# stefantaubert/waveglow

Hardware: AMD Instinct MI355X
Metric: audio samples/sec/GPU (22.05 kHz) WaveGlow-256 infer; real-time factor (higher is better)
Workload: dtype f16 MFMA operands, f32 accumulate/flow state, fp16 I/O; 1 GPU; configs[1]: 256ch WaveGlow.infer, batch=16/GPU mels 80x864, fp16 I/O, sigma=0.6; parallelism=utterance-sharded x1, no collective

## Files before the change

### waveglow_amd/csrc/kernels.hip

```cpp
#include "wg_common.h"

#include <cstdlib>
#include <type_traits>

namespace wg {

typedef _Float16 half8 __attribute__((ext_vector_type(8)));
typedef _Float16 half4 __attribute__((ext_vector_type(4)));
typedef float f32x16 __attribute__((ext_vector_type(16)));
typedef float f32x4 __attribute__((ext_vector_type(4)));

#define WG_GPTR(p) ((const __attribute__((address_space(1))) void*)(p))
#define WG_LPTR(p) ((__attribute__((address_space(3))) void*)(p))

__device__ __forceinline__ float load_io(const void* p, size_t i, int f16) {
  return f16 ? (float)((const _Float16*)p)[i] : ((const float*)p)[i];
}

__device__ __forceinline__ float gate_act(float u, float v) {
  const float e1 = __builtin_amdgcn_exp2f(__builtin_amdgcn_fmed3f(u, -60.0f, 60.0f));
  const float t = 1.0f + __builtin_amdgcn_exp2f(v);
  return (e1 - 1.0f) * __builtin_amdgcn_rcpf(fmaf(e1, t, t));
}

__device__ __forceinline__ void gate_act3(float u, float v, float& th, float& sg, float& ac) {
  const float e1 = __builtin_amdgcn_exp2f(__builtin_amdgcn_fmed3f(u, -60.0f, 60.0f));
  const float t = 1.0f + __builtin_amdgcn_exp2f(__builtin_amdgcn_fmed3f(v, -60.0f, 60.0f));
  const float r = __builtin_amdgcn_rcpf(fmaf(e1, t, t));
  ac = fmaf(e1, r, -r);
  sg = fmaf(e1, r, r);
  th = ac * t;
}

__device__ __forceinline__ void glds16(const void* sbase, unsigned voff, unsigned lds_addr) {
  unsigned keep;
  asm volatile("s_mov_b32 %0, m0\n\ts_mov_b32 m0, %3\n\ts_nop 2\n\tglobal_load_lds_dwordx4 %1, %2\n\ts_mov_b32 m0, %0"
               : "=&s"(keep) : "v"(voff), "s"(sbase), "s"(lds_addr) : "memory");
}
template <int OFF>
__device__ __forceinline__ void gload16(half8& dst, const void* sbase, unsigned voff) {
  asm volatile("s_nop 4\n\tglobal_load_dwordx4 %0, %1, %2 offset:%3" : "=v"(dst) : "v"(voff), "s"(sbase), "i"(OFF) : "memory");
}

#ifdef WG_STAMPS
#define WG_STAMP(i)                                                                              \
  do {                                                                                           \
    __builtin_amdgcn_sched_barrier(0);                                                           \
    unsigned long long _t;                                                                       \
    asm volatile("s_memtime %0\n\ts_waitcnt lgkmcnt(0)" : "=s"(_t)::"memory");                   \
    if (a.stamps && HAS_RES && tid == 0) a.stamps[(size_t)tile * 8 + (i)] = _t;                        \
    __builtin_amdgcn_sched_barrier(0);                                                           \
  } while (0)
#else
#define WG_STAMP(i) do {} while (0)
#endif

constexpr int kTilesPerWG = 2;


__device__ __forceinline__ void mfma16_acc(f32x4& c, const half8& a, const half8& b) {
  c = __builtin_amdgcn_mfma_f32_16x16x32_f16(a, b, c, 0, 0, 0);
}

template <int C> struct WnCfg {
  static constexpr int NW = (C >= 256) ? 8 : C / 32;
  static constexpr int BN = (C >= 512) ? 64 : 128;
};

template <int N> __device__ __forceinline__ void wait_vm() {
  asm volatile("s_waitcnt vmcnt(%0)" :: "i"(N) : "memory");
  __builtin_amdgcn_sched_barrier(0);
}

template <int C, int NW, int BN, bool HAS_RES, int TPW, int CX, int MODE = 0, int NTAPS = 3, bool HAS_COND = true, bool DEEP = false, bool M16 = false>
__global__ void __launch_bounds__(NW * 64) wn_layer_kernel(const WnLayerArgs a) {
  constexpr bool TR = MODE == 1;
  constexpr bool PLAIN = MODE >= 2;
  constexpr int MB = C / (32 * NW);
  constexpr int MT = PLAIN ? MB : 2 * MB;
  constexpr int NTHREADS = NW * 64;
  constexpr int NT = BN / 32;
  constexpr int CC = CX;
  constexpr int NKX = NTAPS * CC;
  constexpr int BT_BYTES = BN * 128;
  constexpr int ACT_ROW = 2 * C + 16;
  constexpr int K2 = C / 16;
  constexpr int NG = BN * 8 / NTHREADS;
  constexpr int NAH = MT * 2;
  constexpr bool DEFER = (MB == 1);
  static_assert(BN * 8 % NTHREADS == 0 && MB >= 1 && MB <= 2 && NKX >= 1 && (NTAPS == 1 || NTAPS == 3), "tile geometry");
  constexpr bool Q2L = !M16 && DEFER && !DEEP && (NG + NT - 1) / NT == 1 && NT >= NG + MT;
  static_assert(!M16 || (MODE == 0 && MB == 1 && DEFER && !DEEP && NT >= 2), "16x16x32 variant");
  constexpr bool A0G = MODE == 0 && CX == 1 && NTAPS == 1;
  static_assert(!DEEP || (MODE == 0 && DEFER && HAS_COND && MT <= NT && NG <= NT && ((NKX >= 4 && NKX % 2 == 0) || NKX == 1)), "deep prefetch variant");
  static_assert(MODE == 0 || (TPW == 1 && CX == ((MODE == 2 || MODE == 4) ? 2 : 1) * (C / 64)) || (MODE == 3 && CX == 1), "training variants");

  extern __shared__ __attribute__((aligned(16))) char smem[];
  char* const sB = smem;
  char* const sActs = MODE == 4 ? smem : smem + 2 * BT_BYTES;

  const int tid = threadIdx.x;
  const int wave = __builtin_amdgcn_readfirstlane(tid >> 6);
  int lane = tid & 63, ln = lane & 31, lh = lane >> 5;

  unsigned pvoff[NG];
  int pchunk[NG];
  int swB;
  int l15 = lane & 15, l4 = lane >> 4;
  unsigned a_voff;
  auto set_lane_ids = [&]() {
    int t = tid;
    asm volatile("" : "+v"(t));
    lane = t & 63;
    ln = lane & 31;
    lh = lane >> 5;
    swB = M16 ? (lane >> 1) & 7 : (ln >> 1) & 7;
    l15 = lane & 15;
    l4 = lane >> 4;
    a_voff = lane * 16;
#pragma unroll
    for (int i = 0; i < NG; ++i) {
      const int idx = i * NTHREADS + t;
      const int row = idx >> 3, pc = idx & 7;
      pchunk[i] = pc ^ ((row >> 1) & 7);
      pvoff[i] = row * 128 + (pchunk[i] << 4);
    }
  };
  set_lane_ids();
  const unsigned sB_addr = (unsigned)(size_t)WG_LPTR(sB);
  const int R = a.g.R, Rp = a.g.Rp, Fp = a.g.Fp, M = a.M;
  const int nK = NKX + (HAS_COND ? a.n_cond_steps : 0);
  const int mel_rows_per_utt = a.g.T + 6;

  auto xstep_src = [&](int p, int jt, int ks) -> const char* {
    const int tap = ks / CC, cc = ks - tap * CC;
    const int pp = p + (tap - NTAPS / 2) * a.dil;
    const int row = kRowPad + (pp & 31) * Rp + a.row0 + jt * BN + (pp >> 5);
    return (const char*)(a.x_tap + ((size_t)cc * R + row) * 64);
  };
  auto sp_src = [&](int p, int jt, int s_) -> const char* {
    const int row = kRowPad + p * Rp + a.row0 + jt * BN;
    return (const char*)(a.sp + ((size_t)s_ * R + row) * 64);
  };
  int mrow[NG];
  auto cond_voff = [&](int s, int i) -> unsigned {
    const int k0 = s * 64 + pchunk[i] * 8;
    const int j = (k0 >= M) + (k0 >= 2 * M) + (k0 >= 3 * M);
    return (unsigned)(((mrow[i] - j) * M + (k0 - j * M)) * 2);
  };
  auto stage_B_piece = [&](int p, int jt, int ks, int bufsel, int i) {
    const unsigned lds = __builtin_amdgcn_readfirstlane(sB_addr + bufsel * BT_BYTES + (i * NTHREADS + wave * 64) * 16);
    if constexpr (A0G) {
      if (ks < NKX) {
        const int row = (i * NTHREADS + tid) >> 3, lc = pchunk[i];
        const int pp = p + ((lc < 3 ? lc : 1) - 1) * a.dil;
        const unsigned prow = (unsigned)(kRowPad + (pp & 31) * Rp + a.row0 + jt * BN + (pp >> 5) + row);
        glds16(a.x_tap, prow * 128u + (lc < 3 ? 0u : (unsigned)lc * 16u), lds);
        return;
      }
    }
    if (ks < NKX) glds16(xstep_src(p, jt, ks), pvoff[i], lds);
    else if constexpr (MODE != 0) glds16(sp_src(p, jt, ks - NKX), pvoff[i], lds);
    else glds16(a.melT, cond_voff(ks - NKX, i), lds);
  };
  auto read_B = [&](const char* buf, int nt, int k16) -> half8 {
    const int n = nt * 32 + ln;
    const int c = (k16 * 2 + lh) ^ swB;
    return *(const half8*)(buf + n * 128 + c * 16);
  };
  auto read_B16 = [&](const char* buf, int g, int nt) -> half8 {
    const int n = (NT * (g & 1) + nt) * 16 + l15;
    const int c = (4 * (g >> 1) + l4) ^ swB;
    return *(const half8*)(buf + n * 128 + c * 16);
  };
  const char* wA1c_p = nullptr;
  auto load_Aq = [&](int ks, int g, int mt, half8& dst) {
    const char* base = ks < NKX ? (const char*)a.wA1 : wA1c_p;
    const int kl = ks < NKX ? ks : ks - NKX;
    const char* p = base + ((size_t)(2 * kl + (g >> 1)) * NW + wave) * (NAH * 1024) + (mt * 2 + (g & 1)) * 1024;
    gload16<0>(dst, p, a_voff);
  };
  auto load_A16 = [&](int ks, int s_, int m, half8& dst) {
    const char* base = ks < NKX ? (const char*)a.wA1 : wA1c_p;
    const int kl = ks < NKX ? ks : ks - NKX;
    gload16<0>(dst, base + ((size_t)(2 * kl + s_) * NW + wave) * (NAH * 1024) + m * 1024, a_voff);
  };
  int tile_b0 = 0;
  const bool fp_ge_bn = Fp >= BN;
  auto column_of = [&](int rr, int p, int& b, int& t) -> bool {
    int rem = rr - tile_b0 * Fp;
    b = tile_b0;
    if (fp_ge_bn) {
      if (rem >= Fp) { rem -= Fp; ++b; }
    } else {
      const int qd = rem / Fp;
      b += qd;
      rem -= qd * Fp;
    }
    const int fq = rem - a.g.Gf;
    t = fq * 32 + p;
    if (!(b < a.g.B && fq >= 0 && fq < a.g.F && t < a.g.L)) return false;
    return a.g.frames == nullptr || t < 32 * a.g.frames[b];
  };

  int tile, tile_end;
  const int tile_step = gridDim.x >> 3;
  int run_start, run_quarter = 0;
  {
    const int bid = blockIdx.x, ntl = a.n_tiles;
    const int xcd = bid & 7, idx = bid >> 3;
    const int qq = ntl >> 3, r = ntl & 7;
    const int start = xcd < r ? xcd * (qq + 1) : r * (qq + 1) + (xcd - r) * qq;
    tile_end = start + (xcd < r ? qq + 1 : qq);
    tile = start + idx;
    run_start = start;
    if (((tile_end - start) & 3) == 0) run_quarter = (tile_end - start) >> 2;
  }
  auto tile_of = [&](int t) { return run_quarter ? run_start + ((t - run_start) & 3) * run_quarter + ((t - run_start) >> 2) : t; };

  half8 q[4][MT];
  int par = 0;
  if (tile < tile_end) {
    const int t0 = tile_of(tile), p0 = t0 / a.tiles_per_phase;
#pragma unroll
    for (int i = 0; i < NG; ++i) stage_B_piece(p0, t0 - p0 * a.tiles_per_phase, 0, 0, i);
  }
  float* const sBias = (float*)(sActs + BN * ACT_ROW);
  if constexpr (!PLAIN) {
    for (int i = tid; i < 2 * C; i += NTHREADS) sBias[i] = a.bias1[i];
    if constexpr (HAS_RES)
      for (int i = tid; i < C; i += NTHREADS) sBias[2 * C + i] = a.bias2[i];
    uint4* const sW = (uint4*)(sBias + 3 * C);
    for (int i = tid; i < (C / 32) * 64; i += NTHREADS) sW[i] = ((const uint4*)a.wEs)[i];
  }
  __syncthreads();

#pragma unroll
  for (int it = 0; it < TPW; ++it, tile += tile_step) {
    if (tile >= tile_end) break;
    if (it > 0) set_lane_ids();
    const int tile_m = tile_of(tile);
    const int p = tile_m / a.tiles_per_phase;
    const int jt = tile_m - p * a.tiles_per_phase;
    const int rr0 = a.row0 + jt * BN;
    tile_b0 = rr0 / Fp;
    const int r0 = kRowPad + p * Rp + rr0;
    const int next_tile = tile + tile_step;
    wA1c_p = (const char*)a.wA1c + (MODE != 0 ? (size_t)0 : (size_t)p * (2 * a.n_cond_steps) * NW * (NAH * 1024));
    half8 Q[DEEP ? 2 : 1][4][MT];
    if constexpr (DEEP) {
#pragma unroll
      for (int g = 0; g < 4; ++g)
#pragma unroll
        for (int mt = 0; mt < MT; ++mt) load_Aq(0, g, mt, Q[0][g][mt]);
#pragma unroll
      for (int g = 0; g < 2; ++g)
#pragma unroll
        for (int mt = 0; mt < MT; ++mt) load_Aq(1, g, mt, Q[DEEP ? 1 : 0][g][mt]);
    } else {
#pragma unroll
      for (int g = 0; g < (Q2L || M16 ? 2 : 3); ++g)
#pragma unroll
        for (int mt = 0; mt < MT; ++mt) {
          if constexpr (M16) load_A16(0, 0, 2 * g + mt, q[g][mt]);
          else load_Aq(0, g, mt, q[g][mt]);
        }
    }
    if constexpr (MODE == 0) {
#pragma unroll
      for (int i = 0; i < NG; ++i) {
        int b, t;
        const int rr = rr0 + ((i * NTHREADS + tid) >> 3);
        const bool ok = column_of(rr, p, b, t);
        mrow[i] = ok ? 3 + b * mel_rows_per_utt + 3 + (t >> 5) : 3;
      }
    }
    unsigned vmask = 0;
#pragma unroll
    for (int nt = 0; nt < NT; ++nt) {
      int cb, ct;
      vmask |= column_of(rr0 + nt * 32 + ln, p, cb, ct) ? (1u << nt) : 0u;
    }
    WG_STAMP(0);
    f32x16 acc[MT][NT];
    f32x4 acc4[M16 ? MT : 1][M16 ? NT : 1][4];
    auto acc_at = [&](int mt, int nt, int e) -> float {
      if constexpr (M16) return acc4[mt][nt][e >> 2][e & 3];
      else return acc[mt][nt][e];
    };
#pragma unroll
    for (int mt = 0; mt < MT; ++mt) {
      f32x16 v;
      if constexpr (PLAIN) {
#pragma unroll
        for (int j = 0; j < 16; ++j) v[j] = 0.0f;
      } else {
        const int row0 = (mt < MB ? 0 : C) + (wave * MB + (mt < MB ? mt : mt - MB)) * 32;
        const float4* bp = (const float4*)(sBias + row0 + 4 * (M16 ? l4 : lh));
#pragma unroll
        for (int g = 0; g < 4; ++g) {
          const float4 q4 = bp[M16 ? 4 * (g >> 1) : 2 * g];
          v[4 * g] = q4.x; v[4 * g + 1] = q4.y; v[4 * g + 2] = q4.z; v[4 * g + 3] = q4.w;
        }
      }
#pragma unroll
      for (int nt = 0; nt < NT; ++nt) {
        if constexpr (M16) {
#pragma unroll
          for (int e = 0; e < 4; ++e) acc4[mt][nt][e] = f32x4{v[4 * e], v[4 * e + 1], v[4 * e + 2], v[4 * e + 3]};
        } else {
          acc[mt][nt] = v;
        }
      }
    }

    constexpr bool PIPE = !PLAIN && HAS_RES && MB == 1;
    constexpr bool RES_A0 = A0G && wn_res_a0(C);
    half8 a2r[PIPE ? K2 : 1];
    wait_vm<DEEP ? 3 * MT : 0>();
    __builtin_amdgcn_s_barrier();
    __builtin_amdgcn_sched_barrier(0);
    WG_STAMP(1);
    constexpr int LPS = (MT + NT - 1) / NT;
    constexpr int GPS = (NG + NT - 1) / NT;
    half8 bf[2][NT];
    constexpr bool PRIO = NW == 8 && ((BN == 128 && ((MODE == 0 && CX == C / 64) || MODE == 1)) || (C == 512 && MODE == 0 && CX == C / 64));
    auto prio_set = [&](int hi_grp) {
      if (hi_grp == 1)
        asm volatile("s_cmp_lt_u32 %0, 4\n\ts_cbranch_scc1 .Lpa%=\n\ts_setprio 1\n\ts_branch .Lpb%=\n.Lpa%=:\n\ts_setprio 0\n.Lpb%=:" :: "s"(wave) : "memory", "scc");
      else
        asm volatile("s_cmp_lt_u32 %0, 4\n\ts_cbranch_scc1 .Lpa%=\n\ts_setprio 0\n\ts_branch .Lpb%=\n.Lpa%=:\n\ts_setprio 1\n.Lpb%=:" :: "s"(wave) : "memory", "scc");
    };
    auto mfma_col = [&](int g, int nt) {
      if constexpr (M16) {
        const int t16 = NT * (g & 1) + nt;
#pragma unroll
        for (int m = 0; m < 4; ++m) {
          mfma16_acc(acc4[m >> 1][t16 >> 1][2 * (m & 1) + (t16 & 1)], q[2 * (g >> 1) + (m >> 1)][m & 1], bf[g & 1][nt]);
        }
      } else {
#pragma unroll
        for (int mt = 0; mt < MT; ++mt) {
          acc[mt][nt] = __builtin_amdgcn_mfma_f32_32x32x16_f16(q[g][mt], bf[g & 1][nt], acc[mt][nt], 0, 0, 0);
        }
      }
    };
    auto kstep = [&](auto more_tag, auto ncond_tag, auto first_tag, int ks) {
      constexpr bool more = decltype(more_tag)::value;
      constexpr bool ncond = decltype(ncond_tag)::value;
      constexpr bool first = decltype(first_tag)::value;
      const char* buf = sB + ((ks + par) & 1) * BT_BYTES;
      const char* src_next = nullptr;
      if constexpr (more && !ncond) src_next = xstep_src(p, jt, ks + 1);
      if constexpr (more && ncond && MODE != 0) src_next = sp_src(p, jt, ks + 1 - NKX);
      const unsigned lds_next = sB_addr + ((ks + 1 + par) & 1) * BT_BYTES + wave * 1024;
#pragma unroll
      for (int nt = 0; nt < NT; ++nt) bf[0][nt] = M16 ? read_B16(buf, 0, nt) : read_B(buf, nt, 0);
      __builtin_amdgcn_sched_barrier(0);
      auto dma_slot = [&](int nt) {
        if constexpr (more) {
#pragma unroll
          for (int i = nt * GPS; i < (nt + 1) * GPS && i < NG; ++i) {
            const unsigned lds = __builtin_amdgcn_readfirstlane(lds_next + i * NTHREADS * 16);
            if constexpr (ncond && MODE == 0) glds16(a.melT, cond_voff(ks + 1 - NKX, i), lds);
            else glds16(src_next, pvoff[i], lds);
          }
        }
      };
      if constexpr (PRIO) {
        prio_set(1);
        __builtin_amdgcn_sched_barrier(0);
      }
      if constexpr (DEFER) {
#pragma unroll
        for (int nt = 0; nt < NT; ++nt) {
          if constexpr (!first) mfma_col(3, nt);
          __builtin_amdgcn_sched_barrier(0);
          dma_slot(nt);
          if constexpr (Q2L) {
            if (nt >= NG && nt - NG < MT) load_Aq(ks, 2, nt - NG, q[2][nt - NG]);
          }
          __builtin_amdgcn_sched_barrier(0);
        }
      }
#pragma unroll
      for (int g = 0; g < (DEFER ? 3 : 4); ++g) {
        if constexpr (M16) {
          if (g == 0) wait_vm<more ? NG : 0>();
          if (g == 2) wait_vm<0>();
        } else {
        if (g == 1) wait_vm<more ? 2 * MT + NG : 2 * MT>();
        if (g == 2) wait_vm<Q2L ? (more ? 2 * MT : MT) : (more ? NG + 2 * MT : MT)>();
        if (g == 3) wait_vm<more ? 2 * MT : 0>();
        }
#pragma unroll
        for (int nt = 0; nt < NT; ++nt) {
          mfma_col(g, nt);
          __builtin_amdgcn_sched_barrier(0);
          if (g < 3) bf[(g + 1) & 1][nt] = M16 ? read_B16(buf, g + 1, nt) : read_B(buf, nt, g + 1);
          if (!DEFER && g == 0) dma_slot(nt);
          if constexpr (M16) {
            constexpr int LP16 = (4 + NT - 1) / NT;
            if (g == 0 || (g == 2 && more)) {
#pragma unroll
              for (int m = nt * LP16; m < (nt + 1) * LP16 && m < 4; ++m)
                load_A16(g == 0 ? ks : ks + 1, g == 0 ? 1 : 0, m, q[(g == 0 ? 2 : 0) + (m >> 1)][m & 1]);
            }
          } else if (g == 0 || more) {
#pragma unroll
            for (int mt = nt * LPS; mt < (nt + 1) * LPS && mt < MT; ++mt)
              load_Aq(g == 0 ? ks : ks + 1, (g + 3) & 3, mt, q[(g + 3) & 3][mt]);
          }
          if constexpr (PRIO) {
            if (g == 0 && nt == NT - 1) prio_set(0);
          }
          __builtin_amdgcn_sched_barrier(0);
        }
      }
      if constexpr (more) {
        if constexpr (DEFER && !Q2L && !M16) {
#pragma unroll
          for (int mt = 0; mt < MT; ++mt) load_Aq(ks + 1, 2, mt, q[2][mt]);
        }
        asm volatile("s_waitcnt vmcnt(%0) lgkmcnt(0)" :: "i"(M16 ? 4 : Q2L ? MT : 2 * MT) : "memory");
        __builtin_amdgcn_s_barrier();
        __builtin_amdgcn_sched_barrier(0);
      }
    };
    auto kstep_d = [&](auto par_tag, auto more_tag, auto more2_tag, auto ncond_tag, auto first_tag, int ks) {
      constexpr int P = DEEP ? decltype(par_tag)::value : 0, PO = DEEP ? 1 - P : 0;
      constexpr bool more = decltype(more_tag)::value, more2 = decltype(more2_tag)::value;
      constexpr bool ncond = decltype(ncond_tag)::value, first = decltype(first_tag)::value;
      const char* buf = sB + ((ks + par) & 1) * BT_BYTES;
      const char* src_next = nullptr;
      if constexpr (more && !ncond) src_next = xstep_src(p, jt, ks + 1);
      const unsigned lds_next = sB_addr + ((ks + 1 + par) & 1) * BT_BYTES + wave * 1024;
#pragma unroll
      for (int nt = 0; nt < NT; ++nt) bf[0][nt] = read_B(buf, nt, 0);
      __builtin_amdgcn_sched_barrier(0);
#pragma unroll
      for (int nt = 0; nt < NT; ++nt) {
        if constexpr (!first) {
#pragma unroll
          for (int mt = 0; mt < MT; ++mt)
            acc[mt][nt] = __builtin_amdgcn_mfma_f32_32x32x16_f16(Q[PO][3][mt], bf[1][nt], acc[mt][nt], 0, 0, 0);
        }
        __builtin_amdgcn_sched_barrier(0);
        if constexpr (more) {
          if (nt < NG) {
            const unsigned lds = __builtin_amdgcn_readfirstlane(lds_next + nt * NTHREADS * 16);
            if constexpr (ncond) glds16(a.melT, cond_voff(ks + 1 - NKX, nt), lds);
            else glds16(src_next, pvoff[nt], lds);
          }
          if (nt == NT - 1) {
#pragma unroll
            for (int mt = 0; mt < MT; ++mt) load_Aq(ks + 1, 2, mt, Q[PO][2][mt]);
          }
        }
        __builtin_amdgcn_sched_barrier(0);
      }
#pragma unroll
      for (int g = 0; g < 3; ++g) {
#pragma unroll
        for (int nt = 0; nt < NT; ++nt) {
#pragma unroll
          for (int mt = 0; mt < MT; ++mt)
            acc[mt][nt] = __builtin_amdgcn_mfma_f32_32x32x16_f16(Q[P][g][mt], bf[g & 1][nt], acc[mt][nt], 0, 0, 0);
          __builtin_amdgcn_sched_barrier(0);
          bf[(g + 1) & 1][nt] = read_B(buf, nt, g + 1);
          if (nt < MT) {
            if (g == 0 && more) load_Aq(ks + 1, 3, nt, Q[PO][3][nt]);
            if (g >= 1 && more2) load_Aq(ks + 2, g - 1, nt, Q[P][g - 1][nt]);
          }
          __builtin_amdgcn_sched_barrier(0);
        }
      }
      if constexpr (more) {
        asm volatile("s_waitcnt vmcnt(%0) lgkmcnt(0)" :: "i"(more2 ? 3 * MT : MT) : "memory");
        __builtin_amdgcn_s_barrier();
        __builtin_amdgcn_sched_barrier(0);
      }
    };
    if constexpr (DEEP) {
      using T_ = std::true_type;
      using F_ = std::false_type;
      using P0 = std::integral_constant<int, 0>;
      using P1 = std::integral_constant<int, 1>;
      if constexpr (NKX == 1) {
        kstep_d(P0{}, T_{}, T_{}, T_{}, T_{}, 0);
        kstep_d(P1{}, T_{}, T_{}, T_{}, F_{}, 1);
        kstep_d(P0{}, T_{}, T_{}, T_{}, F_{}, 2);
        kstep_d(P1{}, T_{}, T_{}, T_{}, F_{}, 3);
        kstep_d(P0{}, T_{}, F_{}, T_{}, F_{}, 4);
        kstep_d(P1{}, F_{}, F_{}, F_{}, F_{}, 5);
      } else {
        kstep_d(P0{}, T_{}, T_{}, F_{}, T_{}, 0);
#pragma clang loop unroll(disable)
        for (int ks = 1; ks < NKX - 1; ks += 2) {
          kstep_d(P1{}, T_{}, T_{}, F_{}, F_{}, ks);
          kstep_d(P0{}, T_{}, T_{}, F_{}, F_{}, ks + 1);
        }
        kstep_d(P1{}, T_{}, T_{}, T_{}, F_{}, NKX - 1);
        kstep_d(P0{}, T_{}, T_{}, T_{}, F_{}, NKX);
        kstep_d(P1{}, T_{}, T_{}, T_{}, F_{}, NKX + 1);
        kstep_d(P0{}, T_{}, T_{}, T_{}, F_{}, NKX + 2);
        kstep_d(P1{}, T_{}, F_{}, T_{}, F_{}, NKX + 3);
        kstep_d(P0{}, F_{}, F_{}, F_{}, F_{}, NKX + 4);
      }
      constexpr int PL = (NKX + 4) & 1;
      wait_vm<0>();
#pragma unroll
      for (int nt = 0; nt < NT; ++nt)
#pragma unroll
        for (int mt = 0; mt < MT; ++mt)
          acc[mt][nt] = __builtin_amdgcn_mfma_f32_32x32x16_f16(Q[DEEP ? PL : 0][3][mt], bf[1][nt], acc[mt][nt], 0, 0, 0);
    }
    if constexpr (!DEEP) {
      using T_ = std::true_type;
      using F_ = std::false_type;
      if constexpr (NKX == 1) {
        if constexpr (HAS_COND) kstep(T_{}, T_{}, T_{}, 0);
        else kstep(F_{}, F_{}, T_{}, 0);
      } else {
        kstep(T_{}, F_{}, T_{}, 0);
#pragma clang loop unroll(disable)
        for (int ks = 1; ks < NKX - 1; ++ks) kstep(T_{}, F_{}, F_{}, ks);
        if constexpr (HAS_COND) kstep(T_{}, T_{}, F_{}, NKX - 1);
        else kstep(F_{}, F_{}, F_{}, NKX - 1);
      }
      if constexpr (HAS_COND) {
#pragma clang loop unroll(disable)
        for (int ks = NKX; ks < nK - 1; ++ks) kstep(T_{}, T_{}, F_{}, ks);
        kstep(F_{}, F_{}, F_{}, nK - 1);
      }
    }
    if constexpr (DEFER && !DEEP) {
      wait_vm<0>();
#pragma unroll
      for (int nt = 0; nt < NT; ++nt) mfma_col(3, nt);
    }
    if constexpr (PRIO) asm volatile("s_setprio 0" ::: "memory");
    __builtin_amdgcn_sched_barrier(0);
    par = (par + nK) & 1;
    if (next_tile < tile_end) {
      const int tn = tile_of(next_tile), pn = tn / a.tiles_per_phase;
#pragma unroll
      for (int i = 0; i < NG; ++i) stage_B_piece(pn, tn - pn * a.tiles_per_phase, 0, par, i);
    }
    __builtin_amdgcn_sched_barrier(0);

    WG_STAMP(2);
    if constexpr (PLAIN) {
      auto gate_derivative = [&](const f32x16& g, const _Float16* tp, const _Float16* sp_, _Float16* dst, size_t off) {
        const half8 t0 = *(const half8*)(tp + off), t1 = *(const half8*)(tp + off + 8);
        const half8 s0 = *(const half8*)(sp_ + off), s1 = *(const half8*)(sp_ + off + 8);
        half8 o0, o1, p0, p1;
#pragma unroll
        for (int r = 0; r < 8; ++r) {
          const float ta = (float)t0[r], sa = (float)s0[r], ga = g[r];
          const float tb = (float)t1[r], sb = (float)s1[r], gb = g[8 + r];
          o0[r] = (_Float16)(ga * sa * (1.0f - ta * ta));
          o1[r] = (_Float16)(gb * sb * (1.0f - tb * tb));
          p0[r] = (_Float16)(ga * ta * sa * (1.0f - sa));
          p1[r] = (_Float16)(gb * tb * sb * (1.0f - sb));
        }
        const size_t off_s = off + (size_t)(C / 64) * R * 64;
        *(half8*)(dst + off) = o0;
        *(half8*)(dst + off + 8) = o1;
        *(half8*)(dst + off_s) = p0;
        *(half8*)(dst + off_s + 8) = p1;
      };
      int lno = ln, lho = lh;
      if constexpr (MODE == 4) {
        asm volatile("" : "+v"(lno), "+v"(lho));
        __syncthreads();
      }
#pragma unroll
      for (int nt = 0; nt < NT; ++nt) {
        int cb, ct;
        const bool col_ok = column_of(rr0 + nt * 32 + ln, p, cb, ct);
        if (MODE != 4 && !col_ok) continue;
#pragma unroll
        for (int mb = 0; mb < MB; ++mb) {
          const int blk = wave * MB + mb;
          const size_t off = ((size_t)(blk >> 1) * R + r0 + nt * 32 + ln) * 64 + (blk & 1) * 32 + lh * 16;
          if constexpr (MODE == 2 || MODE == 4) {
            half8 i0, i1, o0, o1;
            if (a.in0) { i0 = *(const half8*)(a.in0 + off); i1 = *(const half8*)(a.in0 + off + 8); }
#pragma unroll
            for (int r = 0; r < 8; ++r) {
              o0[r] = (_Float16)(acc[mb][nt][r] + (a.in0 ? (float)i0[r] : 0.0f));
              o1[r] = (_Float16)(acc[mb][nt][8 + r] + (a.in0 ? (float)i1[r] : 0.0f));
            }
            if (col_ok) {
              *(half8*)(a.out0 + off) = o0;
              *(half8*)(a.out0 + off + 8) = o1;
            }
            if constexpr (MODE == 4) {
              if (!col_ok) {
#pragma unroll
                for (int r = 0; r < 8; ++r) { o0[r] = (_Float16)0.0f; o1[r] = (_Float16)0.0f; }
              }
              char* ap = sActs + lno * ACT_ROW + lho * 32 + nt * 32 * ACT_ROW + blk * 64;
              *(half8*)(ap) = o0;
              *(half8*)(ap + 16) = o1;
            }
          } else {
            gate_derivative(acc[mb][nt], a.in0, a.in1, a.out0, off);
          }
        }
      }
      if constexpr (MODE == 4) {
        __syncthreads();
        __builtin_amdgcn_sched_barrier(0);
        constexpr int KX = C / 16;
        auto a_frag = [&](int mb, int k) -> half8 {
          const size_t e = ((((size_t)(k >> 2) * 2 + ((k >> 1) & 1)) * NW + wave) * MB + mb) * 2 + (k & 1);
          return *((const half8*)a.wat_prev + e * 64 + lane);
        };
        f32x16 acc2[MB][NT];
#pragma unroll
        for (int mb = 0; mb < MB; ++mb)
#pragma unroll
          for (int nt = 0; nt < NT; ++nt)
#pragma unroll
            for (int j = 0; j < 16; ++j) acc2[mb][nt][j] = 0.0f;
        constexpr int PF4 = 4;
        half8 af[MB][PF4];
#pragma unroll
        for (int mb = 0; mb < MB; ++mb)
#pragma unroll
          for (int i = 0; i < PF4; ++i) af[mb][i] = a_frag(mb, i);
        half8 go[NT];
#pragma unroll
        for (int nt = 0; nt < NT; ++nt) go[nt] = *(const half8*)(a.gout + ((size_t)r0 + nt * 32 + lno) * 64 + lho * 8);
        const char* const acts_rd = sActs + lno * ACT_ROW + lho * 16;
        half8 bq[2][NT];
#pragma unroll
        for (int nt = 0; nt < NT; ++nt) bq[0][nt] = *(const half8*)(acts_rd + nt * 32 * ACT_ROW);
#pragma unroll
        for (int k = 0; k < KX; ++k) {
          if (k + 1 < KX) {
#pragma unroll
            for (int nt = 0; nt < NT; ++nt) bq[(k + 1) & 1][nt] = *(const half8*)(acts_rd + nt * 32 * ACT_ROW + (k + 1) * 32);
          }
#pragma unroll
          for (int mb = 0; mb < MB; ++mb) {
            const half8 afk = af[mb][k % PF4];
            if (k + PF4 < KX) af[mb][k % PF4] = a_frag(mb, k + PF4);
#pragma unroll
            for (int nt = 0; nt < NT; ++nt)
              acc2[mb][nt] = __builtin_amdgcn_mfma_f32_32x32x16_f16(afk, bq[k & 1][nt], acc2[mb][nt], 0, 0, 0);
          }
        }
#pragma unroll
        for (int mb = 0; mb < MB; ++mb) {
          const half8 afo = a_frag(mb, 4 * (C / 64));
#pragma unroll
          for (int nt = 0; nt < NT; ++nt)
            acc2[mb][nt] = __builtin_amdgcn_mfma_f32_32x32x16_f16(afo, go[nt], acc2[mb][nt], 0, 0, 0);
        }
#pragma unroll
        for (int nt = 0; nt < NT; ++nt) {
          int cb, ct;
          if (!column_of(rr0 + nt * 32 + lno, p, cb, ct)) continue;
#pragma unroll
          for (int mb = 0; mb < MB; ++mb) {
            const int blk = wave * MB + mb;
            const size_t off = ((size_t)(blk >> 1) * R + r0 + nt * 32 + lno) * 64 + (blk & 1) * 32 + lho * 16;
            gate_derivative(acc2[mb][nt], a.t_prev, a.s_prev, a.dpre_prev, off);
          }
        }
      }
    }
    if constexpr (!PLAIN) {
    int lno = ln, lho = lh, laneo = lane;
    asm volatile("" : "+v"(lno), "+v"(lho), "+v"(laneo));
    char* const acts_lane = sActs + lno * ACT_ROW + lho * 32;
    const char* const acts_rd = sActs + lno * ACT_ROW + lho * 16;
    const int l15 = laneo & 15, l4 = laneo >> 4;
    char* const acts_lane16 = sActs + l15 * ACT_ROW + (l4 & 1) * 32 + (l4 >> 1) * 8;
    auto write_acts16 = [&](int c, int blk_, int mh, const half8& o) {
      typedef _Float16 half4_t __attribute__((ext_vector_type(4)));
      const half4_t lo = {o[0], o[1], o[2], o[3]}, hi = {o[4], o[5], o[6], o[7]};
      char* ap = acts_lane16 + c * 32 * ACT_ROW + blk_ * 64 + mh * 16;
      *(half4_t*)(ap) = lo;
      *(half4_t*)(ap + 16 * ACT_ROW) = hi;
    };
    constexpr int NGRP = (BN / 16 + NW - 1) / NW;
    constexpr bool kWesEarly = (C / 32) * 4 <= 32;
    half8 wes[C / 32];
    float4 es_o[NGRP];
    float4* es_op[NGRP];
    bool es_valid[NGRP];
    auto es_prefetch_w = [&](int s_) { wes[s_] = ((const half8*)(sBias + 3 * C) + laneo)[s_ * 64]; };
    auto es_prefetch = [&]() {
#pragma unroll
      for (int gi = 0; gi < NGRP; ++gi) {
        const int grp = wave + gi * NW;
        es_valid[gi] = false;
        es_o[gi] = make_float4(0.f, 0.f, 0.f, 0.f);
        es_op[gi] = nullptr;
        if (grp < BN / 16) {
          int cb, ct;
          es_valid[gi] = column_of(rr0 + grp * 16 + l15, p, cb, ct) && laneo < 32;
          es_op[gi] = (float4*)(a.out + ((size_t)cb * a.g.L + ct) * 8 + 4 * l4);
          if (es_valid[gi]) es_o[gi] = *es_op[gi];
        }
      }
    };
    auto es_compute = [&]() {
#pragma unroll
      for (int s = 0; s < C / 32; ++s) es_prefetch_w(s);
#pragma unroll
      for (int gi = 0; gi < NGRP; ++gi) {
        const int grp = wave + gi * NW;
        if (grp < BN / 16) {
          const char* ep = sActs + (grp * 16 + l15) * ACT_ROW + l4 * 16;
          f32x4 d = {0.f, 0.f, 0.f, 0.f};
#pragma unroll
          for (int s = 0; s < C / 32; ++s) {
            const half8 bfe = *(const half8*)(ep + s * 64);
            d = __builtin_amdgcn_mfma_f32_16x16x32_f16(wes[s], bfe, d, 0, 0, 0);
          }
#pragma unroll
          for (int r = 0; r < 4; ++r) d[r] += __shfl_xor(d[r], 32);
          if (es_valid[gi]) {
            float4 o = es_o[gi];
            o.x += d[0]; o.y += d[1]; o.z += d[2]; o.w += d[3];
            *es_op[gi] = o;
          }
        }
      }
    };
    auto read_acts32 = [&](int nt, int k16) -> half8 {
      return *(const half8*)(acts_rd + nt * 32 * ACT_ROW + k16 * 32);
    };
    constexpr int PF = 8 / MB;
    half8 xres[RES_A0 ? 1 : MB][RES_A0 ? 1 : NT][2];
    half8 a0f[RES_A0 ? NT : 1], wst[RES_A0 ? MB : 1];
    half8 a2[MB][PF];
    const half8* const p2 = (const half8*)a.wA2 + (size_t)wave * MB * K2 * 64 + laneo;
    f32x16 acc2[MB][NT];
    if constexpr (PIPE) {
      constexpr int SL = 16;
      const int blk = wave;
      const float* const sBias2 = sBias + 2 * C;
      half8 idA[RES_A0 ? 1 : 2];
      if constexpr (RES_A0) {
        idA[0] = ((const half8*)a.wStA)[blk * 64 + laneo];
      } else {
        const int pr = 16 * ((lno >> 2) & 1) + 4 * (lno >> 3) + (lno & 3);
#pragma unroll
        for (int sx = 0; sx < 2; ++sx)
#pragma unroll
          for (int j = 0; j < 8; ++j) idA[sx][j] = (_Float16)((16 * sx + 8 * lho + j) == pr ? 1.0f : 0.0f);
      }
      half8 xr[RES_A0 ? 1 : 2];
      auto load_xr = [&](int nt) {
        if constexpr (RES_A0) {
          xr[0] = *(const half8*)(a.x_tap + ((size_t)r0 + nt * 32 + lno) * 64 + lho * 8);
        } else {
          const size_t row = (size_t)(blk >> 1) * R + r0 + nt * 32 + lno;
          const half8* xp = (const half8*)(a.x_in + row * 64 + (blk & 1) * 32 + lho * 8);
          xr[0] = xp[0];
          xr[1] = xp[2];
        }
      };
      load_xr(0);
      half8* const xo_base = (half8*)(a.x_out + ((size_t)(blk >> 1) * R + r0 + lno) * 64 + (blk & 1) * 32 + lho * 16);
      auto store_xout_half = [&](const f32x16& d, int nt, int hf) {
        if ((vmask >> nt) & 1u) {
          half8 qv;
#pragma unroll
          for (int r = 0; r < 8; ++r) qv[r] = (_Float16)d[8 * hf + r];
          xo_base[(size_t)nt * 32 * 8 + hf] = qv;
        }
      };
      __builtin_amdgcn_sched_barrier(0);
      auto phase = [&](auto c_tag) {
        constexpr int c = decltype(c_tag)::value;
        constexpr bool do_gate = c < NT, do_mm = c >= 1;
        f32x16 d2;
        if (do_mm) {
          const float4* bp = (const float4*)(sBias2 + blk * 32 + 4 * lho);
#pragma unroll
          for (int g = 0; g < 4; ++g) {
            const float4 b4 = bp[2 * g];
            d2[4 * g + 0] = b4.x;
            d2[4 * g + 1] = b4.y;
            d2[4 * g + 2] = b4.z;
            d2[4 * g + 3] = b4.w;
          }
          d2 = __builtin_amdgcn_mfma_f32_32x32x16_f16(idA[0], xr[0], d2, 0, 0, 0);
          if constexpr (!RES_A0) d2 = __builtin_amdgcn_mfma_f32_32x32x16_f16(idA[1], xr[1], d2, 0, 0, 0);
        }
        if (do_mm && c < NT) load_xr(c);
        if (c == NT - 1) es_prefetch();
        if (c == NT) es_compute();
        float e1[SL], den[SL], rc[SL];
        half8 o0, o1, th0, th1, sg0, sg1;
        auto stageA = [&](int e) {
          const int nt = c < NT ? c : 0;
          const float u = __builtin_amdgcn_fmed3f(acc_at(0, nt, e), -60.0f, 60.0f);
          e1[e] = __builtin_amdgcn_exp2f(u);
          den[e] = __builtin_amdgcn_exp2f(TR ? __builtin_amdgcn_fmed3f(acc_at(MB, nt, e), -60.0f, 60.0f) : acc_at(MB, nt, e));
        };
        auto stageB = [&](int e) {
          const float t = 1.0f + den[e];
          rc[e] = __builtin_amdgcn_rcpf(fmaf(e1[e], t, t));
          if constexpr (TR) den[e] = t;
        };
        auto stageC = [&](int e) {
          float v = fmaf(e1[e], rc[e], -rc[e]);
          asm volatile("" : "+v"(v));
          if (e < 8) o0[e] = (_Float16)v; else o1[e - 8] = (_Float16)v;
          if constexpr (TR) {
            float sg = fmaf(e1[e], rc[e], rc[e]), th = v * den[e];
            asm volatile("" : "+v"(sg), "+v"(th));
            if (e < 8) { sg0[e] = (_Float16)sg; th0[e] = (_Float16)th; } else { sg1[e - 8] = (_Float16)sg; th1[e - 8] = (_Float16)th; }
          }
        };
        bool save_ok = false;
        size_t save_off = 0;
        if constexpr (TR) {
          if (do_gate) {
            save_ok = (vmask >> c) & 1u;
            save_off = ((size_t)(blk >> 1) * R + r0 + c * 32 + lno) * 64 + (blk & 1) * 32 + lho * 16;
          }
        }
        static_assert(K2 <= SL, "one GEMM-2 MFMA per slot at most");
        half8 bq[K2];
        const int ntm = c >= 1 ? c - 1 : 0;
        auto k_of = [](int i) { return i * K2 / SL; };
        auto has_k = [&](int i) { return i >= 0 && i < SL && k_of(i) != k_of(i + 1); };
        if (do_gate) { stageA(0); stageA(1); stageB(0); }
        if (do_mm) {
          if (has_k(0)) bq[k_of(0)] = read_acts32(ntm, k_of(0));
          if (has_k(1)) bq[k_of(1)] = read_acts32(ntm, k_of(1));
        }
        __builtin_amdgcn_sched_barrier(0);
#pragma unroll
        for (int i = 0; i < SL; ++i) {
          if (do_mm) {
            if (has_k(i + 2)) bq[k_of(i + 2)] = read_acts32(ntm, k_of(i + 2));
            if (has_k(i)) d2 = __builtin_amdgcn_mfma_f32_32x32x16_f16(a2r[k_of(i)], bq[k_of(i)], d2, 0, 0, 0);
          }
          if (c == 0 && i < K2) a2r[i] = p2[(size_t)i * 64];
          if (do_gate) {
            if (i + 2 < SL) stageA(i + 2);
            if (i + 1 < SL) stageB(i + 1);
            if (i & 1) { stageC(i - 1); stageC(i); }
            if constexpr (M16) {
              if (i == 7) write_acts16(c, blk, 0, o0);
              if (i == SL - 1) write_acts16(c, blk, 1, o1);
            } else {
              if (i == 7) *(half8*)(acts_lane + c * 32 * ACT_ROW + blk * 64) = o0;
              if (i == SL - 1) *(half8*)(acts_lane + c * 32 * ACT_ROW + blk * 64 + 16) = o1;
            }
            if constexpr (TR) {
              if (i == 7 && save_ok) {
                *(half8*)(a.save_a + save_off) = o0;
                *(half8*)(a.save_t + save_off) = th0;
                *(half8*)(a.save_s + save_off) = sg0;
              }
              if (i == SL - 1 && save_ok) {
                *(half8*)(a.save_a + save_off + 8) = o1;
                *(half8*)(a.save_t + save_off + 8) = th1;
                *(half8*)(a.save_s + save_off + 8) = sg1;
              }
            }
          }
          __builtin_amdgcn_sched_barrier(0);
        }
        if (do_mm) {
          store_xout_half(d2, ntm, 0);
          store_xout_half(d2, ntm, 1);
        }
        if (do_gate) {
          asm volatile("s_waitcnt lgkmcnt(0)" ::: "memory");
          __builtin_amdgcn_s_barrier();
          asm volatile("" ::: "memory");
          __builtin_amdgcn_sched_barrier(0);
          if (c == 0) WG_STAMP(3);
          if (c == 1) WG_STAMP(5);
          if (c == 2) WG_STAMP(6);
          if (c == 3) WG_STAMP(7);
        }
      };
      phase(std::integral_constant<int, 0>{});
      phase(std::integral_constant<int, 1>{});
      if constexpr (NT >= 2) phase(std::integral_constant<int, 2>{});
      if constexpr (NT >= 3) phase(std::integral_constant<int, 3>{});
      if constexpr (NT >= 4) phase(std::integral_constant<int, 4>{});
      static_assert(NT <= 4, "phases are instantiated explicitly");
      WG_STAMP(4);
    }
    if constexpr (!PIPE) {
    if constexpr (HAS_RES) {
      if constexpr (RES_A0) {
#pragma unroll
        for (int nt = 0; nt < NT; ++nt) a0f[nt] = *(const half8*)(a.x_tap + ((size_t)r0 + nt * 32 + lno) * 64 + lho * 8);
#pragma unroll
        for (int mb = 0; mb < MB; ++mb) wst[mb] = ((const half8*)a.wStA)[(wave * MB + mb) * 64 + laneo];
      }
#pragma unroll
      for (int mb = 0; mb < MB; ++mb) {
        const int blk = wave * MB + mb;
        if constexpr (!RES_A0) {
#pragma unroll
          for (int nt = 0; nt < NT; ++nt) {
            const size_t row = (size_t)(blk >> 1) * R + r0 + nt * 32 + lno;
            const half8* xp = (const half8*)(a.x_in + row * 64 + (blk & 1) * 32 + lho * 16);
            xres[mb][nt][0] = xp[0];
            xres[mb][nt][1] = xp[1];
          }
        }
#pragma unroll
        for (int i = 0; i < PF; ++i) a2[mb][i] = p2[((size_t)mb * K2 + i) * 64];
      }
    }
    __builtin_amdgcn_sched_barrier(0);

#pragma unroll
    for (int mb = 0; mb < MB; ++mb) {
#pragma unroll
      for (int nt = 0; nt < NT; ++nt) {
        half8 o0, o1;
        if constexpr (TR) {
          half8 th0, th1, sg0, sg1;
#pragma unroll
          for (int r = 0; r < 8; ++r) {
            float th, sg, ac;
            gate_act3(acc[mb][nt][r], acc[MB + mb][nt][r], th, sg, ac);
            o0[r] = (_Float16)ac; th0[r] = (_Float16)th; sg0[r] = (_Float16)sg;
            gate_act3(acc[mb][nt][8 + r], acc[MB + mb][nt][8 + r], th, sg, ac);
            o1[r] = (_Float16)ac; th1[r] = (_Float16)th; sg1[r] = (_Float16)sg;
          }
          int cb, ct;
          if (column_of(rr0 + nt * 32 + lno, p, cb, ct)) {
            const int blk = wave * MB + mb;
            const size_t off = ((size_t)(blk >> 1) * R + r0 + nt * 32 + lno) * 64 + (blk & 1) * 32 + lho * 16;
            *(half8*)(a.save_a + off) = o0; *(half8*)(a.save_a + off + 8) = o1;
            *(half8*)(a.save_t + off) = th0; *(half8*)(a.save_t + off + 8) = th1;
            *(half8*)(a.save_s + off) = sg0; *(half8*)(a.save_s + off + 8) = sg1;
          }
        } else {
#pragma unroll
          for (int r = 0; r < 8; ++r) {
            o0[r] = (_Float16)gate_act(acc_at(mb, nt, r), acc_at(MB + mb, nt, r));
            o1[r] = (_Float16)gate_act(acc_at(mb, nt, 8 + r), acc_at(MB + mb, nt, 8 + r));
          }
        }
        if constexpr (M16) {
          write_acts16(nt, wave * MB + mb, 0, o0);
          write_acts16(nt, wave * MB + mb, 1, o1);
        } else {
          char* ap = acts_lane + nt * 32 * ACT_ROW + (wave * MB + mb) * 64;
          *(half8*)(ap) = o0;
          *(half8*)(ap + 16) = o1;
        }
      }
    }
    __syncthreads();
    __builtin_amdgcn_sched_barrier(0);
    WG_STAMP(3);

    if constexpr (HAS_RES) {
#pragma unroll
      for (int mb = 0; mb < MB; ++mb) {
        const float* bp = a.bias2 + (wave * MB + mb) * 32 + 4 * lho;
        float bv[16];
#pragma unroll
        for (int r = 0; r < 16; ++r) bv[r] = bp[(r & 3) + 8 * (r >> 2)];
#pragma unroll
        for (int nt = 0; nt < NT; ++nt) {
          if constexpr (RES_A0) {
#pragma unroll
            for (int r = 0; r < 16; ++r) acc2[mb][nt][r] = bv[r];
            acc2[mb][nt] = __builtin_amdgcn_mfma_f32_32x32x16_f16(wst[mb], a0f[nt], acc2[mb][nt], 0, 0, 0);
          } else {
#pragma unroll
            for (int r = 0; r < 8; ++r) {
              acc2[mb][nt][r] = (float)xres[mb][nt][0][r] + bv[r];
              acc2[mb][nt][8 + r] = (float)xres[mb][nt][1][r] + bv[8 + r];
            }
          }
        }
      }
    }

    }


    if constexpr (kWesEarly && !PIPE) es_prefetch();

    if constexpr (HAS_RES && !PIPE) {
      half8 bq[2][NT];
#pragma unroll
      for (int nt = 0; nt < NT; ++nt) bq[0][nt] = read_acts32(nt, 0);
#pragma unroll
      for (int k = 0; k < K2; ++k) {
        if (k + 1 < K2) {
#pragma unroll
          for (int nt = 0; nt < NT; ++nt) bq[(k + 1) & 1][nt] = read_acts32(nt, k + 1);
        }
#pragma unroll
        for (int mb = 0; mb < MB; ++mb) {
          const half8 af = a2[mb][k % PF];
          if (k + PF < K2) a2[mb][k % PF] = p2[((size_t)mb * K2 + k + PF) * 64];
#pragma unroll
          for (int nt = 0; nt < NT; ++nt)
            acc2[mb][nt] = __builtin_amdgcn_mfma_f32_32x32x16_f16(af, bq[k & 1][nt], acc2[mb][nt], 0, 0, 0);
        }
      }
    }

    if constexpr (!PIPE) {
      WG_STAMP(4);
      if constexpr (!kWesEarly) es_prefetch();
      es_compute();
    }

    if constexpr (!PIPE) WG_STAMP(5);
    if constexpr (HAS_RES && !PIPE) {
#pragma unroll
      for (int nt = 0; nt < NT; ++nt) {
        int cb, ct;
        if (column_of(rr0 + nt * 32 + lno, p, cb, ct)) {
#pragma unroll
          for (int mb = 0; mb < MB; ++mb) {
            const int blk = wave * MB + mb;
            half8 o0, o1;
#pragma unroll
            for (int r = 0; r < 8; ++r) {
              o0[r] = (_Float16)acc2[mb][nt][r];
              o1[r] = (_Float16)acc2[mb][nt][8 + r];
            }
            const size_t row = (size_t)(blk >> 1) * R + r0 + nt * 32 + lno;
            half8* xp = (half8*)(a.x_out + row * 64 + (blk & 1) * 32 + lho * 16);
            xp[0] = o0;
            xp[1] = o1;
          }
        }
      }
    }
    if constexpr (!PIPE) WG_STAMP(6);
    }
    __builtin_amdgcn_sched_barrier(0);
  }
}

template <int C, int BN, bool HAS_RES, int TPW, int CX, int MODE = 0, int NTAPS = 3, bool HAS_COND = true, bool DEEP = false>
static hipError_t launch_wn_tttt(const WnLayerArgs& a, hipStream_t s) {
  constexpr int NW = WnCfg<C>::NW;
  constexpr bool M16 = wn_frag16(C, BN) && MODE == 0 && !DEEP;
  if (M16 != (a.frag16 != 0)) return hipErrorInvalidValue;
  if (MODE == 0 && CX == 1 && NTAPS == 1 && wn_res_a0(C) && HAS_RES && !a.wStA) return hipErrorInvalidValue;
  constexpr int smem = MODE == 4 ? (BN * (2 * C + 16) > 2 * BN * 128 ? BN * (2 * C + 16) : 2 * BN * 128)
                                 : 2 * BN * 128 + (MODE >= 2 ? 0 : BN * (2 * C + 16) + 3 * C * 4 + (C / 32) * 1024);
  static bool attr_done_dev[64] = {};
  int cur_dev = 0;
  if (hipGetDevice(&cur_dev) != hipSuccess || cur_dev < 0 || cur_dev >= 64) cur_dev = 0;
  bool& attr_done = attr_done_dev[cur_dev];
  if (!attr_done) {
    hipError_t e = hipFuncSetAttribute((const void*)wn_layer_kernel<C, NW, BN, HAS_RES, TPW, CX, MODE, NTAPS, HAS_COND, DEEP, M16>,
                                       hipFuncAttributeMaxDynamicSharedMemorySize, smem);
    if (e != hipSuccess) return e;
    attr_done = true;
  }
  const int per_label = ((a.n_tiles + 7) / 8 + TPW - 1) / TPW;
  const int grid = 8 * per_label;
  hipLaunchKernelGGL((wn_layer_kernel<C, NW, BN, HAS_RES, TPW, CX, MODE, NTAPS, HAS_COND, DEEP, M16>), dim3(grid), dim3(NW * 64), smem, s, a);
  return hipGetLastError();
}
template <int C, int BN, bool HAS_RES, int TPW>
static hipError_t launch_wn_ttt(const WnLayerArgs& a, hipStream_t s) {
  if constexpr (C == 256 && BN == 64 && TPW == 1) {
    const char* e = getenv("WG_DISABLE_DEEP");
    if (a.n_cond_steps == 5 && !(e && *e == '1')) {
      if (a.a0_fold) return launch_wn_tttt<C, BN, HAS_RES, TPW, 1, 0, 1, true, true>(a, s);
      return launch_wn_tttt<C, BN, HAS_RES, TPW, C / 64, 0, 3, true, true>(a, s);
    }
  }
  if (a.a0_fold) return a.x_chunks_per_tap == 1 ? launch_wn_tttt<C, BN, HAS_RES, TPW, 1, 0, 1>(a, s) : hipErrorInvalidValue;
  return launch_wn_tttt<C, BN, HAS_RES, TPW, C / 64>(a, s);
}
template <int C, int BN, bool HAS_RES>
static hipError_t launch_wn_tt(const WnLayerArgs& a, hipStream_t s) {
  const int ncu = a.n_cu > 0 ? a.n_cu : 1;
  const int rounds1 = (a.n_tiles + ncu - 1) / ncu;
  const int rounds2 = ((a.n_tiles + kTilesPerWG - 1) / kTilesPerWG + ncu - 1) / ncu * kTilesPerWG;
  if (a.n_tiles >= 2 * kTilesPerWG * ncu && rounds2 <= rounds1) return launch_wn_ttt<C, BN, HAS_RES, kTilesPerWG>(a, s);
  return launch_wn_ttt<C, BN, HAS_RES, 1>(a, s);
}
template <int C>
static hipError_t launch_wn_t(const WnLayerArgs& a, int bn, hipStream_t s) {
  if (bn == 64) return a.has_res ? launch_wn_tt<C, 64, true>(a, s) : launch_wn_tt<C, 64, false>(a, s);
  if constexpr (WnCfg<C>::BN == 128) {
    if (bn == 128) return a.has_res ? launch_wn_tt<C, 128, true>(a, s) : launch_wn_tt<C, 128, false>(a, s);
  }
  return hipErrorInvalidValue;
}

int wn_block_n(int C) {
  switch (C) {
    case 64: return WnCfg<64>::BN;
    case 128: return WnCfg<128>::BN;
    case 256: return WnCfg<256>::BN;
    case 512: return WnCfg<512>::BN;
  }
  return 0;
}
int wn_waves(int C) {
  switch (C) {
    case 64: return WnCfg<64>::NW;
    case 128: return WnCfg<128>::NW;
    case 256: return WnCfg<256>::NW;
    case 512: return WnCfg<512>::NW;
  }
  return 0;
}

template <int C>
static hipError_t launch_wn_train_t(const WnLayerArgs& a, int bn, hipStream_t s) {
  if (bn == 64) return a.has_res ? launch_wn_tttt<C, 64, true, 1, C / 64, 1>(a, s) : launch_wn_tttt<C, 64, false, 1, C / 64, 1>(a, s);
  if constexpr (WnCfg<C>::BN == 128) {
    if (bn == 128) return a.has_res ? launch_wn_tttt<C, 128, true, 1, C / 64, 1>(a, s) : launch_wn_tttt<C, 128, false, 1, C / 64, 1>(a, s);
  }
  return hipErrorInvalidValue;
}
hipError_t launch_wn_layer_train(const WnLayerArgs& a, int C, int bn, hipStream_t s) {
  if (!a.sp || !a.save_t || !a.save_s || !a.save_a || a.x_chunks_per_tap != C / 64) return hipErrorInvalidValue;
  switch (C) {
    case 64: return launch_wn_train_t<64>(a, bn, s);
    case 128: return launch_wn_train_t<128>(a, bn, s);
    case 256: return launch_wn_train_t<256>(a, bn, s);
    case 512: return launch_wn_train_t<512>(a, bn, s);
  }
  return hipErrorInvalidValue;
}

template <int C>
static hipError_t launch_wn_plain_t(const WnLayerArgs& a, int kind, int bn, hipStream_t s) {
  constexpr int CCH = C / 64;
  if constexpr (WnCfg<C>::BN == 128) {
    if (bn == 128) {
      if (kind == 2) return launch_wn_tttt<C, 128, false, 1, 2 * CCH, 2, 3, false>(a, s);
      if (kind == 4) return launch_wn_tttt<C, 128, false, 1, 2 * CCH, 4, 3, false>(a, s);
      if (a.x_chunks_per_tap == 1 && a.n_cond_steps == 0) return launch_wn_tttt<C, 128, false, 1, 1, 3, 1, false>(a, s);
      return launch_wn_tttt<C, 128, false, 1, CCH, 3, 1, true>(a, s);
    }
  }
  if (bn != 64) return hipErrorInvalidValue;
  if (kind == 2) return launch_wn_tttt<C, 64, false, 1, 2 * CCH, 2, 3, false>(a, s);
  if (kind == 4) return launch_wn_tttt<C, 64, false, 1, 2 * CCH, 4, 3, false>(a, s);
  if (a.x_chunks_per_tap == 1 && a.n_cond_steps == 0) return launch_wn_tttt<C, 64, false, 1, 1, 3, 1, false>(a, s);
  return launch_wn_tttt<C, 64, false, 1, CCH, 3, 1, true>(a, s);
}
hipError_t launch_wn_plain(const WnLayerArgs& a, int C, int kind, int bn, hipStream_t s) {
  if ((kind != 2 && kind != 3 && kind != 4) || !a.out0 || !a.x_tap || (kind == 3 && (!a.in0 || !a.in1))) return hipErrorInvalidValue;
  if ((kind == 2 || kind == 4) && (a.x_chunks_per_tap != 2 * (C / 64) || a.n_cond_steps != 0)) return hipErrorInvalidValue;
  if (kind == 4 && (!a.wat_prev || !a.gout || !a.t_prev || !a.s_prev || !a.dpre_prev)) return hipErrorInvalidValue;
  if (kind == 3 && !((a.x_chunks_per_tap == 1 && a.n_cond_steps == 0) || (a.x_chunks_per_tap == C / 64 && a.n_cond_steps == 1 && a.sp)))
    return hipErrorInvalidValue;
  switch (C) {
    case 64: return launch_wn_plain_t<64>(a, kind, bn, s);
    case 128: return launch_wn_plain_t<128>(a, kind, bn, s);
    case 256: return launch_wn_plain_t<256>(a, kind, bn, s);
    case 512: return launch_wn_plain_t<512>(a, kind, bn, s);
  }
  return hipErrorInvalidValue;
}

hipError_t launch_wn_layer(const WnLayerArgs& a, int C, int bn, hipStream_t s) {
  switch (C) {
    case 64: return launch_wn_t<64>(a, bn, s);
    case 128: return launch_wn_t<128>(a, bn, s);
    case 256: return launch_wn_t<256>(a, bn, s);
    case 512: return launch_wn_t<512>(a, bn, s);
// ... 386 lines not shown
```

Baseline: 79.44 million samples/s.

## Split gate and GEMM-2 work into opposite-order wave roles in fused WN phase

For the 8-wave, BN=128 mode-0 configuration, each middle phase no longer interleaves gate activations and GEMM-2 MFMAs slot by slot inside every wave. Half the waves now run the gate block first and the MFMA block second, and the other half use the reverse order. The aim is for one half's transcendental VALU work to overlap the other half's MFMA work across waves instead of relying on fine-grained interleave within a wave. Lane indices are also remapped to a direct 32-lane row mapping under this mode. The change risks reshuffling register pressure and LDS access patterns, and relies on the existing per-phase barrier to keep the two orders correct.

```diff
diff --git a/waveglow_amd/csrc/kernels.hip b/waveglow_amd/csrc/kernels.hip
--- a/waveglow_amd/csrc/kernels.hip
+++ b/waveglow_amd/csrc/kernels.hip
@@ -315,6 +315,7 @@
     }
 
     constexpr bool PIPE = !PLAIN && HAS_RES && MB == 1;
+    constexpr bool ROLES = PIPE && MODE == 0 && BN == 128 && !DEEP && NW == 8;
     constexpr bool RES_A0 = A0G && wn_res_a0(C);
     half8 a2r[PIPE ? K2 : 1];
     wait_vm<DEEP ? 3 * MT : 0>();
@@ -676,6 +677,10 @@
     if constexpr (!PLAIN) {
     int lno = ln, lho = lh, laneo = lane;
     asm volatile("" : "+v"(lno), "+v"(lho), "+v"(laneo));
+    if constexpr (ROLES) {
+      lno = laneo & 31;
+      lho = laneo >> 5;
+    }
     char* const acts_lane = sActs + lno * ACT_ROW + lho * 32;
     const char* const acts_rd = sActs + lno * ACT_ROW + lho * 16;
     const int l15 = laneo & 15, l4 = laneo >> 4;
@@ -781,8 +786,9 @@
       auto phase = [&](auto c_tag) {
         constexpr int c = decltype(c_tag)::value;
         constexpr bool do_gate = c < NT, do_mm = c >= 1;
+        constexpr bool split = ROLES && do_gate && do_mm;
         f32x16 d2;
-        if (do_mm) {
+        auto mm_init = [&]() {
           const float4* bp = (const float4*)(sBias2 + blk * 32 + 4 * lho);
 #pragma unroll
           for (int g = 0; g < 4; ++g) {
@@ -794,8 +800,9 @@
           }
           d2 = __builtin_amdgcn_mfma_f32_32x32x16_f16(idA[0], xr[0], d2, 0, 0, 0);
           if constexpr (!RES_A0) d2 = __builtin_amdgcn_mfma_f32_32x32x16_f16(idA[1], xr[1], d2, 0, 0, 0);
-        }
-        if (do_mm && c < NT) load_xr(c);
+          if (c < NT) load_xr(c);
+        };
+        if (do_mm && !split) mm_init();
         if (c == NT - 1) es_prefetch();
         if (c == NT) es_compute();
         float e1[SL], den[SL], rc[SL];
@@ -834,20 +841,16 @@
         const int ntm = c >= 1 ? c - 1 : 0;
         auto k_of = [](int i) { return i * K2 / SL; };
         auto has_k = [&](int i) { return i >= 0 && i < SL && k_of(i) != k_of(i + 1); };
-        if (do_gate) { stageA(0); stageA(1); stageB(0); }
-        if (do_mm) {
+        auto gate_head = [&]() { stageA(0); stageA(1); stageB(0); };
+        auto mm_head = [&]() {
           if (has_k(0)) bq[k_of(0)] = read_acts32(ntm, k_of(0));
           if (has_k(1)) bq[k_of(1)] = read_acts32(ntm, k_of(1));
-        }
-        __builtin_amdgcn_sched_barrier(0);
-#pragma unroll
-        for (int i = 0; i < SL; ++i) {
-          if (do_mm) {
-            if (has_k(i + 2)) bq[k_of(i + 2)] = read_acts32(ntm, k_of(i + 2));
-            if (has_k(i)) d2 = __builtin_amdgcn_mfma_f32_32x32x16_f16(a2r[k_of(i)], bq[k_of(i)], d2, 0, 0, 0);
-          }
-          if (c == 0 && i < K2) a2r[i] = p2[(size_t)i * 64];
-          if (do_gate) {
+        };
+        auto mm_slot = [&](int i) {
+          if (has_k(i + 2)) bq[k_of(i + 2)] = read_acts32(ntm, k_of(i + 2));
+          if (has_k(i)) d2 = __builtin_amdgcn_mfma_f32_32x32x16_f16(a2r[k_of(i)], bq[k_of(i)], d2, 0, 0, 0);
+        };
+        auto gate_slot = [&](int i) {
             if (i + 2 < SL) stageA(i + 2);
             if (i + 1 < SL) stageB(i + 1);
             if (i & 1) { stageC(i - 1); stageC(i); }
@@ -870,12 +873,52 @@
                 *(half8*)(a.save_s + save_off + 8) = sg1;
               }
             }
-          }
-          __builtin_amdgcn_sched_barrier(0);
-        }
-        if (do_mm) {
+        };
+        auto mm_store = [&]() {
           store_xout_half(d2, ntm, 0);
           store_xout_half(d2, ntm, 1);
+        };
+        if constexpr (split) {
+          auto gate_block = [&]() {
+            gate_head();
+            __builtin_amdgcn_sched_barrier(0);
+#pragma unroll
+            for (int i = 0; i < SL; ++i) {
+              gate_slot(i);
+              __builtin_amdgcn_sched_barrier(0);
+            }
+          };
+          auto mm_block = [&]() {
+            mm_init();
+            mm_head();
+            __builtin_amdgcn_sched_barrier(0);
+#pragma unroll
+            for (int i = 0; i < SL; ++i) {
+              mm_slot(i);
+              __builtin_amdgcn_sched_barrier(0);
+            }
+            mm_store();
+            __builtin_amdgcn_sched_barrier(0);
+          };
+          if (wave < NW / 2) {
+            gate_block();
+            mm_block();
+          } else {
+            mm_block();
+            gate_block();
+          }
+        } else {
+          if (do_gate) gate_head();
+          if (do_mm) mm_head();
+          __builtin_amdgcn_sched_barrier(0);
+#pragma unroll
+          for (int i = 0; i < SL; ++i) {
+            if (do_mm) mm_slot(i);
+            if (c == 0 && i < K2) a2r[i] = p2[(size_t)i * 64];
+            if (do_gate) gate_slot(i);
+            __builtin_amdgcn_sched_barrier(0);
+          }
+          if (do_mm) mm_store();
         }
         if (do_gate) {
           asm volatile("s_waitcnt lgkmcnt(0)" ::: "memory");
```

Result: slower. 78.49 million samples/s (-1.2%).
